# Justin900429/autonomous_driving_with_diffusion_model

Hardware: AMD Instinct MI355X
Metric: denoising-steps/sec (higher is better)
Workload: dtype f32

## Files before the change

### autonomous_driving_with_diffusion_model_amd/_lib.py

```python
from __future__ import annotations

import ctypes as C
import os
from typing import Optional, Sequence

import torch

_HERE = os.path.dirname(os.path.abspath(__file__))
LIB_PATH = os.environ.get("ADX_LIB") or os.path.join(_HERE, "libadx.so")

c_f32p = C.POINTER(C.c_float)
i32, i64, f32, vp = C.c_int32, C.c_int64, C.c_float, C.c_void_p


class TConvDesc(C.Structure):
    _fields_ = [("kind", i32), ("taps", i32), ("stride", i32), ("pad", i32), ("c0", i32), ("c1", i32),
                ("cout", i32), ("lin", i32), ("lout", i32), ("groups", i32), ("eps", f32), ("w_layout", i32),
                ("w_flip", i32), ("exact", i32), ("lin_valid", i32), ("lout_valid", i32)]


class TConvIO(C.Structure):
    _fields_ = [("x0", vp), ("x0_sb", i64), ("x0_sc", i64), ("x0_sl", i64),
                ("x1", vp), ("x1_sb", i64), ("x1_sc", i64), ("x1_sl", i64),
                ("packed_w", vp), ("bias", vp), ("gamma", vp), ("beta", vp),
# ... 204 lines not shown
    "adx_control_reset": (i32, [vp, i32, i32, i32, vp, vp]),
    "adx_traj_metrics": (i32, [C.POINTER(MetricsCfg), vp, vp, vp, vp, vp, vp, vp, vp, vp, vp, vp]),
    "adx_metrics_state_bytes": (C.c_size_t, []),
    "adx_metrics_reset": (i32, [vp, vp]),
    "adx_metrics_accumulate": (i32, [vp, vp, vp, vp, vp, vp, vp, i32, i32, vp]),
    "adx_noise_normal": (i32, [vp, i32, i64, vp, i64, vp]),
    "adx_noise_words": (i32, [vp, i32, i64, vp, i64, vp]),
    "adx_noise_advance": (i32, [vp, vp]),
    "adx_warm_init": (i32, [vp, i32, vp, vp, i32, i32, i32, i32, f32, f32, vp, i64, i32, vp]),
    "adx_add_noise": (i32, [vp, vp, vp, vp, vp, i32, vp, i32, i32, i32, i32, vp]),
}

_LAZY_SIGS = {
    "adx_resnet_plan_grids": (i32, [vp, i32, i32, i32, i32, i32, i32, C.POINTER(i32), C.POINTER(i32), i32]),
    "adx_conv2d_hs3x3q_walk": (i32, [i32, i32, i32, C.POINTER(i32), C.POINTER(i32)]),
    "adx_conv2d_pack_ds": (i32, [i32, i32, vp, vp, vp]),
    "adx_conv2d_block_s2_cells": (i32, [i32, i32, vp, vp, vp, vp, vp, vp, vp, vp, vp, i32, i32, i32, i32, vp]),
    "adx_ddim_step_pin": (i32, [C.POINTER(StepCoef), vp, vp, vp, vp, i32, i64, C.POINTER(PinDesc), vp, vp, i32, i32, i32, vp]),
    "adx_ddpm_step_pin": (i32, [C.POINTER(StepCoef), vp, vp, vp, vp, i32, i64, C.POINTER(PinDesc), vp, vp, i32, i32, i32, vp]),
    "adx_dpm_step_pin": (i32, [C.POINTER(DpmCoef), vp, vp, vp, vp, i32, i64, C.POINTER(PinDesc), vp, vp, i32, i32, i32, vp]),
    "adx_pin_apply": (i32, [vp, C.POINTER(PinDesc), vp, i64, i32, i32, i32, vp]),
    "adx_cost_field_from_occupancy": (i32, [vp, vp, i32, i32, i32, f32, f32, f32, i32, i32, vp]),
    "adx_capsules_from_boxes": (i32, [vp, vp, i32, i32, f32, vp]),
    "adx_stop_short": (i32, [vp, C.POINTER(GuideDesc), C.POINTER(FieldDesc), C.POINTER(RouteDesc), C.POINTER(CapsuleDesc), vp, i32, vp, vp,
                             vp, vp, vp, i32, i32, i32, vp]),
    "adx_traj_modes": (i32, [C.POINTER(ModesCfg), vp, vp, vp, vp, vp, vp, vp, vp]),
    "adx_commit_state_bytes": (C.c_size_t, [i32, i32]),
    "adx_commit_reset": (i32, [vp, i32, i32, vp, vp]),
    "adx_traj_commit": (i32, [C.POINTER(CommitCfg), vp, vp, vp, vp, vp, vp, vp, vp, vp, vp, vp, vp, vp]),
}
# ... 116 lines not shown
```

### autonomous_driving_with_diffusion_model_amd/csrc/adx_common.h

```cpp
#pragma once
#include <atomic>
#include <mutex>
#include <hip/hip_runtime.h>
#include <stdint.h>
#include <stdio.h>
#include <string.h>

#include "../../include/adx.h"
#include "plan.h"

namespace adx {

void set_error(const char* fmt, ...);

#define ADX_CHECK_HIP(expr)                                                              \
  do {                                                                                   \
    hipError_t _e = (expr);                                                              \
    if (_e != hipSuccess) {                                                              \
      adx::set_error("%s failed: %s (%s:%d)", #expr, hipGetErrorString(_e), __FILE__, __LINE__); \
      return ADX_ERR_HIP;                                                                \
    }                                                                                    \
  } while (0)

#define ADX_REQUIRE(cond, ...)                                                           \
// ... 15 lines not shown

struct DebugSwitches {
  bool conv_exact = false;
  bool wgrad_exact = false;
  bool tconv_exact = false;
  bool unet_chain = true;
  unsigned chain_mask = ~0u;
  bool unet_pipe = true;
  bool conv_vrow = true;
  bool conv_cells = true;
  int train_cells = 5;
  int hs_mode = -1;
  bool wgrad_deterministic = false;
  bool hs_dma = true;
  bool hs_s2q = true;
  bool hs_persist = true;
  int hs_reserve_cus = -1;
  int hs_grid_cap = 0;
  int resnet_streams = 2;
  int resnet_split_from = -1;
  bool check_range = false;
};
const DebugSwitches& debug_switches();

struct DeviceOnce {
  std::atomic<uint64_t>& done;
  uint64_t bit = 0;
  bool owner = false;
  static std::mutex& mu() { static std::mutex m; return m; }
  explicit DeviceOnce(std::atomic<uint64_t>& d) : done(d) {
// ... 54 lines not shown
```

### autonomous_driving_with_diffusion_model_amd/csrc/api.cpp

```cpp
#include <stdarg.h>
#include <stdlib.h>

#include "sched.h"
#include "tconv.h"

namespace adx {

static thread_local char g_err[512] = "";

void set_error(const char* fmt, ...) {
  va_list ap;
  va_start(ap, fmt);
  vsnprintf(g_err, sizeof(g_err), fmt, ap);
  va_end(ap);
}

static thread_local PlanSink* t_plan_sink = nullptr;
PlanSink* plan_sink() { return t_plan_sink; }
void plan_set_sink(PlanSink* s) { t_plan_sink = s; }

int plan_emit(PlanSink* s, const PlanLaunch& l) {
  ADX_REQUIRE(s->n < s->cap, "plan export: more than %d launches", s->cap);
  s->rec[s->n++] = l;
  return ADX_OK;
// ... 11 lines not shown
const DebugSwitches& debug_switches() {
  static const DebugSwitches sw = [] {
    DebugSwitches d;
    auto is = [](const char* name, char v) { const char* e = getenv(name); return e != nullptr && e[0] == v && e[1] == '\0'; };
    d.conv_exact = is("ADX_CONV_EXACT", '1');
    d.wgrad_exact = is("ADX_WGRAD_EXACT", '1');
    d.tconv_exact = is("ADX_TCONV_EXACT", '1');
    d.unet_chain = !is("ADX_UNET_CHAIN", '0');
    d.unet_pipe = !is("ADX_UNET_PIPE", '0');
    d.conv_cells = !is("ADX_CONV_CELLS", '0');
    d.conv_vrow = !is("ADX_CONV_VROW", '0');
    d.train_cells = is("ADX_TRAIN_CELLS", '0') ? 0 : (is("ADX_TRAIN_CELLS", '1') ? 1 : (is("ADX_TRAIN_CELLS", '2') ? 2 : (is("ADX_TRAIN_CELLS", '3') ? 3 : (is("ADX_TRAIN_CELLS", '4') ? 4 : 5))));
    d.check_range = is("ADX_CHECK_RANGE", '1');
    d.hs_dma = !is("ADX_HS_DMA", '0');
    d.hs_persist = !is("ADX_HS_PERSIST", '0');
    d.hs_s2q = !is("ADX_HS_S2Q", '0');
    d.wgrad_deterministic = is("ADX_WGRAD_DETERMINISTIC", '1');
    if (const char* e = getenv("ADX_CHAIN_MASK")) d.chain_mask = (unsigned)strtoul(e, nullptr, 0);
    if (const char* e = getenv("ADX_HS_MODE")) d.hs_mode = atoi(e);
    if (const char* e = getenv("ADX_HS_RESERVE_CUS")) d.hs_reserve_cus = atoi(e) < 0 ? 0 : (atoi(e) & ~7);
    if (const char* e = getenv("ADX_HS_GRID_CAP")) d.hs_grid_cap = atoi(e) < 8 ? 0 : (atoi(e) & ~7);
    if (const char* e = getenv("ADX_RESNET_SPLIT_FROM")) d.resnet_split_from = atoi(e) < 0 ? -1 : atoi(e);
    if (const char* e = getenv("ADX_RESNET_STREAMS")) d.resnet_streams = atoi(e) < 1 ? 1 : (atoi(e) > 4 ? 4 : atoi(e));
    return d;
  }();
  return sw;
}

int embed_forward(const adx_embed_weights* w, int dim, const int64_t* t, int t_rows, const float* cond,
                  const float* feat, int feat_rows, int rows, float* time_embed, float* mish_cond, hipStream_t s);
// ... 360 lines not shown
```

### autonomous_driving_with_diffusion_model_amd/csrc/conv2d.hip

```cpp
#include <stdlib.h>

#include <vector>

#include "adx_common.h"
#include "conv2d_internal.h"

namespace adx {

constexpr int kCoutT = 64;
constexpr size_t kMaxLds = 96 * 1024;

template <int STRIDE, int K, int ROWS, int CCH = 16>
__global__ void __launch_bounds__(256) conv2d_kernel(const Conv2dArgs a) {
  constexpr int TH = 4 * ROWS;
  constexpr int CC = (K == 7) ? 4 : CCH;
  constexpr int PH = (TH - 1) * STRIDE + K;
  constexpr int PW = (kTileW - 1) * STRIDE + K;
  constexpr int PLANE = PH * PW;
  constexpr int NP = CC * PLANE;
  constexpr int PITEMS = (NP + 255) / 256;
  constexpr int NTAPS = K * K;
  constexpr int NW4 = NTAPS * CC * (kCoutT / 4);
  constexpr int WITEMS = (NW4 + 255) / 256;
  extern __shared__ __attribute__((aligned(16))) float smem[];
// ... 897 lines not shown
  const int Q = grid / 8;
  int n = 0;
  for (int b = 0; b < grid; ++b) {
    const HsQWalk wk = hs3x3q_walk(b & 7, b >> 3, units);
    counts[b] = 0;
    for (int u = wk.first; u < wk.end; u += Q, ++counts[b], ++n) {
      ADX_REQUIRE(n < units, "adx_conv2d_hs3x3q_walk: internal error (more visits than units)");
      const HsQUnit un = hs3x3q_unit(u, cout_tiles);
      visits[2 * n] = un.sp;
      visits[2 * n + 1] = un.ct;
    }
  }
  return ADX_OK;
}

static int resnet_forward_impl(adx_resnet* r, const void* packed, void* workspace, const float* img,
                               const uint8_t* frames_u8, const float* mean, const float* stdv, int32_t batch, int32_t h,
                               int32_t w, float* feature, adx_stream stream);

int adx_resnet_forward(adx_resnet* r, const void* packed, void* workspace, const float* img, int32_t batch, int32_t h,
                       int32_t w, float* feature, adx_stream stream) {
  ADX_REQUIRE(img != nullptr, "adx_resnet_forward: null image");
  return resnet_forward_impl(r, packed, workspace, img, nullptr, nullptr, nullptr, batch, h, w, feature, stream);
}

int adx_resnet_forward_u8(adx_resnet* r, const void* packed, void* workspace, const uint8_t* frames_hwc, const float* mean,
                          const float* stdv, int32_t batch, int32_t h, int32_t w, float* feature, adx_stream stream) {
  ADX_REQUIRE(frames_hwc && mean && stdv, "adx_resnet_forward_u8: null frames / mean / std");
  return resnet_forward_impl(r, packed, workspace, nullptr, frames_hwc, mean, stdv, batch, h, w, feature, stream);
}
// ... 158 lines not shown
```

### autonomous_driving_with_diffusion_model_amd/csrc/conv2d_hs.hip

```cpp
#include <type_traits>
#include <stdlib.h>

#include "adx_common.h"
#include "conv2d_internal.h"
#include "conv2d_hs_common.h"

namespace adx {

template <bool AFFINE = true>
__device__ __forceinline__ void cells_store32(float (&v)[16], const float* sc, const float* sh, int cl0, const float (*res8)[8],
                                              bool relu, __amdgpu_buffer_rsrc_t yrsrc, uint32_t vcell, uint32_t so, uint32_t cplane,
                                              float& amax) {
  float lm = 0.f;
#pragma unroll
  for (int i = 0; i < 2; ++i)
#pragma unroll
    for (int j = 0; j < 4; ++j) {
      const auto sw = __builtin_amdgcn_permlane32_swap(f2u(v[8 * i + j]), f2u(v[8 * i + 4 + j]), false, false);
      v[8 * i + j] = u2f(sw[0]);
      v[8 * i + 4 + j] = u2f(sw[1]);
    }
#pragma unroll
  for (int i = 0; i < 2; ++i) {
    float o[8];
// ... 343 lines not shown
  if (threadIdx.x == 0 && blockIdx.x < 16384) g_hs_trace[blockIdx.x * 8 + slot] = __builtin_readcyclecounter();
}
__device__ __forceinline__ void hs_trace_id() {
  if (threadIdx.x == 0 && blockIdx.x < 16384) {
    unsigned hw, xcc;
    asm volatile("s_getreg_b32 %0, hwreg(HW_REG_HW_ID)" : "=s"(hw));
    asm volatile("s_getreg_b32 %0, hwreg(HW_REG_XCC_ID)" : "=s"(xcc));
    g_hs_trace[blockIdx.x * 8 + 7] = ((unsigned long long)xcc << 32) | hw;
  }
}
#define HS_TRACE(slot) hs_trace(slot)
#else
#define HS_TRACE(slot)
#endif

template <int MODE, int STATS = 0, bool XCELLS = false, bool YCELLS = false, bool VR = false>
__global__ void __launch_bounds__(MODE == 0 ? 256 : 512, 2) conv2d_hs3x3_kernel(const Conv2dArgs a) {
  constexpr bool VROW = YCELLS || VR;
  constexpr int NT = MODE == 0 ? 256 : 512;
  constexpr int TH = MODE == 1 ? 16 : 8;
  constexpr int CT = MODE == 2 ? 2 : 1;
  constexpr int K = 3, PH = TH + 2, PW = 34, PLANE = PH * PW, NITEM = 2 * PLANE;
  constexpr int PIT = (NITEM + NT - 1) / NT;
  constexpr int NW = 9 * 256, WST = 3 * 256 * CT;
  constexpr int WIT = (WST + NT - 1) / NT;
  static_assert(PIT <= K, "a patch slice travels with each stage of a chunk");
  extern __shared__ __attribute__((aligned(16))) unsigned char smem_raw[];
  u32x4* patch = reinterpret_cast<u32x4*>(smem_raw);
  u32x4* wl = patch + 2 * 4 * PLANE;
  float* ss = reinterpret_cast<float*>(wl + 2 * WST);
  u32x4* dummy = reinterpret_cast<u32x4*>(ss + 2 * 64 * CT + 8);
  float* bsl = reinterpret_cast<float*>(dummy + 3);
  const int tid = threadIdx.x, lane = tid & 63;
  const int wave = __builtin_amdgcn_readfirstlane(tid >> 6);
  const int rowpair = MODE == 2 ? (wave & 3) : wave, slab = MODE == 2 ? (wave >> 2) : 0;
#ifdef ADX_HS_TRACE
  hs_trace_id();
#endif
  HS_TRACE(0);
// ... 1 lines not shown
  {
    const int per = gridDim.x >> 3;
    if (bid < per * 8) bid = (bid & 7) * per + (bid >> 3);
  }
  int kpart = 0;
  if (a.ksplit > 1) { kpart = bid % a.ksplit; bid /= a.ksplit; }
  const int ct = bid % a.cout_tiles; bid /= a.cout_tiles;
  const int tx = bid % a.tiles_x; bid /= a.tiles_x;
  const int ty = bid % a.tiles_y; bid /= a.tiles_y;
  const int n = VROW ? 0 : bid;
  const int oy0 = ty * TH, ox0 = tx * kTileW;
  const int iy0 = oy0 - a.pad, ix0 = ox0 - a.pad;
  const int cout0 = (ct * CT + slab) * kHsCout;
  const int l31 = lane & 31, khalf = lane >> 5;
  const int vx0 = tx * kTileW;
  const int vl = vx0 + l31;
  auto vdiv = [&](int v) { return (int)(((float)v + 0.5f) * a.inv_vw); };
  const int nl = VROW ? vdiv(vl) : 0, xl = VROW ? vl - nl * a.vw : 0;
  const bool lane_valid = !VROW || (nl < a.N && xl < a.W);
  const size_t hw = (size_t)a.H * a.W;
  const int nchunks_all = a.cin_pad / kHsCC;
  const int nchunks = a.ksplit > 1 ? a.cper : nchunks_all;
  const int chunk0 = kpart * nchunks;
  const float* xin = a.x + ((size_t)n * a.Cin + (size_t)chunk0 * kHsCC) * hw;
  const int nstages = nchunks * K;
  const u32x4* wsrc = reinterpret_cast<const u32x4*>(a.w) + ((size_t)ct * CT * nchunks_all + chunk0) * NW;
  constexpr uint32_t kOutside = 0xC0000000u;
  const __amdgpu_buffer_rsrc_t xrsrc = __builtin_amdgcn_make_buffer_rsrc(
      const_cast<float*>(xin), 0,
      (int)(uint32_t)((VROW ? (size_t)a.N * a.Cin : (size_t)(a.Cin - chunk0 * kHsCC)) * hw * sizeof(float)), 0x00020000);
  const uint32_t plane_bytes = (uint32_t)(hw * sizeof(float));
// ... 67 lines not shown
      xs_inv = __builtin_bit_cast(float, (uint32_t)(127 - sh) << 23);
    }
  }

  f32x16 accm[2][2], accl[2][2];
#pragma unroll
  for (int r = 0; r < 2; ++r)
#pragma unroll
    for (int m = 0; m < 2; ++m)
#pragma unroll
      for (int i = 0; i < 16; ++i) { accm[r][m][i] = 0.f; accl[r][m][i] = 0.f; }

  u32x4 wv[2][WIT];
  float pv[2][8];
  auto load_w = [&](int stage, int set) {
    const u32x4* ws = wsrc + (size_t)stage * 768;
#pragma unroll
    for (int k = 0; k < WIT; ++k) wv[set][k] = ws[wsrc_off[k]];
  };
  auto store_w = [&](int set, int buf) {
#pragma unroll
    for (int k = 0; k < WIT; ++k) {
      u32x4* d = (WST % NT == 0 || wdst[k] >= 0) ? wl + buf * WST + wdst[k] : dummy + 2;
      *d = wv[set][k];
    }
  };
  auto load_p = [&](int chunk, int k, int set) {
    const uint32_t cbase = (uint32_t)chunk * kHsCC * plane_bytes;
    if (XCELLS) {
      const u32x4 h4 = __builtin_amdgcn_raw_buffer_load_b128(xrsrc, goff[k], cbase, 0);
// ... 13 lines not shown
    u32x4 hi, lo;
    if (XCELLS) {
#pragma unroll
      for (int j = 0; j < 4; ++j) {
        hi[j] = __builtin_bit_cast(uint32_t, pv[set][j]);
        lo[j] = __builtin_bit_cast(uint32_t, pv[set][4 + j]);
      }
    } else {
      split8(pv[set], xs, hi, lo);
    }
    u32x4* pd = patch + buf * 4 * PLANE + pcell[k];
    u32x4* d0 = pcell[k] >= 0 ? pd : dummy;
    u32x4* d1 = pcell[k] >= 0 ? pd + PLANE : dummy + 1;
    *d0 = hi;
    *d1 = lo;
  };

  const int pb_lane = khalf * 2 * PLANE + (rowpair * 2) * PW + l31;
  const int wa_lane = slab * 768 + khalf * 64 + l31;

  load_w(0, 0);
  store_w(0, 0);
#pragma unroll
  for (int k = 0; k < PIT; ++k) { load_p(0, k, 0); store_p(0, k, 0); }
  load_w(1, 1);
  if (tid < 2 * 64 * CT) ss[tid] = ssv;
  if (STATS == 2 && tid < 4 * 64 * CT) bsl[tid] = bsv;
  load_p(1, 0, 1);
  HS_TRACE(1);
  __syncthreads();
  HS_TRACE(2);

  for (int cp = 0; cp < nchunks; cp += 2) {
#pragma unroll
    for (int i = 0; i < 6; ++i) {
      const int s = 3 * cp + i;
      const int kh = i % 3, cpar = (i / 3) & 1;
      const u32x4* pb0 = patch + cpar * 4 * PLANE + pb_lane;
      const u32x4* wa0 = wl + (i & 1) * WST + wa_lane;
      load_w(s + 2 < nstages ? s + 2 : nstages - 1, i & 1);
      if ((i + 1) % 3 < PIT) load_p(s + 4 < nstages ? (s + 4) / 3 : nchunks - 1, (i + 1) % 3, i & 1);
      __builtin_amdgcn_sched_barrier(0);
#pragma unroll
      for (int kw = 0; kw < K; ++kw) {
        f16x8 A[2][2], B[2][2];
#pragma unroll
        for (int pl = 0; pl < 2; ++pl) {
// ... 8 lines not shown
          for (int m = 0; m < 2; ++m) {
            accm[r][m] = hs_mfma(A[0][m], B[0][r], accm[r][m]);
            accl[r][m] = hs_mfma(A[0][m], B[1][r], accl[r][m]);
            accl[r][m] = hs_mfma(A[1][m], B[0][r], accl[r][m]);
          }
        if (kw == 0) {
          store_w((i + 1) & 1, (i + 1) & 1);
          if (i % 3 < PIT) store_p((i + 1) & 1, i % 3, ((i + 3) / 3) & 1);
        }
      }
      __syncthreads();
    }
  }

  HS_TRACE(3);
  const int ox = VROW ? xl : ox0 + l31;
  const uint32_t plane_ob = (uint32_t)(a.OH * a.OW) * (uint32_t)sizeof(float);
  const size_t img = (size_t)n * a.Cout * a.OH * a.OW;
  const int img_bytes = (int)(uint32_t)((VROW ? (uint32_t)a.N : 1u) * (uint32_t)a.Cout * plane_ob);
  const uint32_t img_off = VROW ? (uint32_t)nl * (uint32_t)a.Cout * plane_ob : 0u;
  float* const ybase = a.ksplit > 1 ? a.part + (size_t)kpart * a.part_stride : a.y;
  const __amdgpu_buffer_rsrc_t yrsrc = __builtin_amdgcn_make_buffer_rsrc(ybase + img, 0, img_bytes, 0x00020000);
  const __amdgpu_buffer_rsrc_t rrsrc = __builtin_amdgcn_make_buffer_rsrc(
      const_cast<float*>(a.res != nullptr ? a.res + img : a.y), 0, a.res != nullptr ? img_bytes : 0, 0x00020000);
  const float* sst = ss + slab * 64;
  const uint32_t cbase_o = (uint32_t)cout0 * plane_ob;
  const uint32_t cplane = (uint32_t)(a.OH * a.OW) * 16u;
  const uint32_t cell0 = (uint32_t)(cout0 >> 3) * 2u * cplane;
  bool inside[2];
  uint32_t pix[2];
#pragma unroll
  for (int rr = 0; rr < 2; ++rr) {
    const int oy = oy0 + rowpair * 2 + rr;
    inside[rr] = lane_valid && oy < a.OH && ox < a.OW;
    pix[rr] = (uint32_t)(oy * a.OW + ox);
  }
  auto half4 = [](uint32_t h0, uint32_t h1, uint32_t l0, uint32_t l1, float* out) {
    const float inv = 1.f / kLoScale;
    asm("v_fma_mix_f32 %0, %1, %2, %3 op_sel:[0,0,0] op_sel_hi:[1,0,1]" : "=v"(out[0]) : "v"(l0), "s"(inv), "v"(h0));
    asm("v_fma_mix_f32 %0, %1, %2, %3 op_sel:[1,0,1] op_sel_hi:[1,0,1]" : "=v"(out[1]) : "v"(l0), "s"(inv), "v"(h0));
    asm("v_fma_mix_f32 %0, %1, %2, %3 op_sel:[0,0,0] op_sel_hi:[1,0,1]" : "=v"(out[2]) : "v"(l1), "s"(inv), "v"(h1));
    asm("v_fma_mix_f32 %0, %1, %2, %3 op_sel:[1,0,1] op_sel_hi:[1,0,1]" : "=v"(out[3]) : "v"(l1), "s"(inv), "v"(h1));
  };
  float amax = 0.f;
  if constexpr (YCELLS) {
    const uint32_t khoff = (uint32_t)khalf * 2u * cplane;
    uint32_t vcell[2], vres[2];
#pragma unroll
    for (int rr = 0; rr < 2; ++rr) {
      vcell[rr] = inside[rr] ? img_off + pix[rr] * 16u + khoff : kOutside;
      vres[rr] = !inside[rr] ? kOutside : a.res_cells ? vcell[rr] : img_off + pix[rr] * 4u + (uint32_t)(8 * khalf) * plane_ob;
    }
    uint32_t rraw[2][2][2][8];
#pragma unroll
    for (int rr = 0; rr < 2; ++rr)
#pragma unroll
      for (int half = 0; half < 2; ++half)
#pragma unroll
// ... 867 lines not shown
  }
  const float sc = scale != nullptr ? scale[c] : 1.f, sh = shift != nullptr ? shift[c] : 0.f;
  v = v * sc + sh;
  if (res != nullptr) v += reinterpret_cast<const f32x4*>(res)[i];
  if (relu) {
#pragma unroll
    for (int k = 0; k < 4; ++k) v[k] = __builtin_fmaxf(v[k], 0.f);
  }
  reinterpret_cast<f32x4*>(y)[i] = v;
  float amax = 0.f;
#pragma unroll
  for (int k = 0; k < 4; ++k) amax = fp16_amax(amax, v[k]);
  range_flag(status, out_of_fp16(amax));
}

static constexpr size_t hs3x3_lds(int mode, int stats) {
  const int th = mode == 1 ? 16 : 8, ct = mode == 2 ? 2 : 1;
  return (size_t)2 * 64 * (th + 2) * 34 + (size_t)2 * 3 * 256 * ct * 16 + (2 * 64 * ct + 8) * sizeof(float) + 48 +
         (stats == 2 ? 4 * 64 * ct * sizeof(float) : 0);
}
static_assert(hs3x3_lds(0, 2) <= 80 * 1024 && hs3x3_lds(1, 2) <= 160 * 1024 && hs3x3_lds(2, 2) <= 160 * 1024, "LDS budget");

Hs3x3Plan conv2d_hs3x3_plan(const ConvSpec& L, const Hs3x3Query& q, const DebugSwitches& sw) {
  Hs3x3Plan p;
  p.admitted = q.fmt == 0;
  if (!hs_eligible(L, sw) || !(L.k == 3 && L.stride == 1 && L.pad == 1) || (L.cin_pad / kHsCC) % 2 != 0) return p;
  const int N = q.N, OH = q.H, OW = q.W, nchunks = L.cin_pad / kHsCC;
  int mode = L.cin < 256 ? 0 : (OH > 8 ? 1 : (L.cout % 128 == 0 ? 2 : 0));
  const long grid0 = (long)N * ceil_div(OH, 8) * ceil_div(OW, kTileW) * (L.cout / kHsCout);
  if (grid0 <= 256) mode = 0;
  if (sw.hs_mode >= 0 && !(sw.hs_mode == 2 && L.cout % 128 != 0)) mode = sw.hs_mode == 1 || sw.hs_mode == 2 ? sw.hs_mode : 0;
  const int th = mode == 1 ? 16 : 8, ct = mode == 2 ? 2 : 1;
  const bool xc = (q.fmt & kFmtXCells) != 0, yc = (q.fmt & kFmtYCells) != 0, rc = (q.fmt & kFmtResCells) != 0 && q.has_res;
  const bool xscaled = q.x_scale == kXScalePre;
  const bool in_ok = (size_t)N * L.cin * q.H * q.W * sizeof(float) < 0xC0000000u;
  const bool bytes_ok = in_ok && (size_t)N * L.cout * OH * OW * sizeof(float) < 0xC0000000u;
// ... 26 lines not shown
  if (!stats && split_shape && q.split_floats > 0 && q.x_scale == kXScaleNone && (OH * OW) % 4 == 0 && q.y_aligned && (!q.has_res || q.res_aligned)) {
    const size_t out_floats = (size_t)N * L.cout * OH * OW;
    int S = 16;
    while (S > 1 && (nchunks % S != 0 || (nchunks / S) % 2 != 0 || p.grid * S > 256 || out_floats * S > q.split_floats)) S >>= 1;
    if (S > 1) { p.ksplit = S; p.cper = nchunks / S; p.grid *= S; }
  }
  const bool cells_out = !stats && p.ksplit == 1 && (xc || yc || rc) && !(xc && xscaled && !yc && !rc);
  if (stats ? q_train || q_dgrad : cells_out && q_plain) {
    p.family = kHs3x3q; p.dma = sw.hs_dma; p.threads = kQNT;
    p.lds = p.dma ? kQLdsD : kQLds;
    p.vw = vw; p.tiles_x = vtiles_x; p.tiles_y = ceil_div(OH, kQTH); p.cout_tiles = L.cout / 128;
    p.q_slots = hs3x3q_slots(p.cout_tiles * p.tiles_x * p.tiles_y, q.cus, sw.hs_dma && sw.hs_persist);
    p.grid = (size_t)8 * p.q_slots;
    return p;
  }
  p.lds = hs3x3_lds(mode, p.stats);
  if (p.ksplit > 1) return p;
  p.xcells = xc; p.ycells = cells_out;
  p.vr = !cells_out && (!(xc || yc || rc) || ((stats || xscaled) && !yc && !rc)) && vrow_ok;
  if (p.ycells || p.vr) {
    p.vw = vw; p.tiles_x = vtiles_x;
    p.grid = (size_t)p.cout_tiles * p.tiles_x * p.tiles_y;
  }
  return p;
}

typedef void (*HsKernel)(const Conv2dArgs);

template <int MODE>
static const HsKernel* hs3x3_kernels() {
#define HS_K(S, X, Y, V) &conv2d_hs3x3_kernel<MODE, S, X, Y, V>
  static const HsKernel table[3 * 8] = {
      HS_K(0, false, false, false), HS_K(0, false, false, true), HS_K(0, false, true, false), nullptr,
      HS_K(0, true, false, false),  HS_K(0, true, false, true),  HS_K(0, true, true, false),  nullptr,
      HS_K(1, false, false, false), HS_K(1, false, false, true), nullptr, nullptr,
      HS_K(1, true, false, false),  HS_K(1, true, false, true),  nullptr, nullptr,
      HS_K(2, false, false, false), HS_K(2, false, false, true), nullptr, nullptr,
      HS_K(2, true, false, false),  HS_K(2, true, false, true),  nullptr, nullptr};
#undef HS_K
  return table;
}

static int hs3x3_launch(const Hs3x3Plan& p, Conv2dArgs a, hipStream_t s) {
  const HsKernel* const table = p.mode == 1 ? hs3x3_kernels<1>() : (p.mode == 2 ? hs3x3_kernels<2>() : hs3x3_kernels<0>());
  static std::atomic<uint64_t> attr[3];
  if (DeviceOnce once{attr[p.mode]}; once) {
    for (int v = 0; v < 3 * 8; ++v)
      if (table[v] != nullptr)
        ADX_CHECK_HIP(hipFuncSetAttribute(reinterpret_cast<const void*>(table[v]), hipFuncAttributeMaxDynamicSharedMemorySize,
                                          (int)hs3x3_lds(p.mode, v / 8)));
    once.commit();
  }
  ADX_REQUIRE(p.grid < (1u << 31), "conv2d_hs: grid too large");
  ADX_REQUIRE((size_t)a.Cout * a.OH * a.OW * sizeof(float) < 0x7FFFFFFFu, "conv2d_hs: one image of the output exceeds the 32-bit byte offsets");
  if (p.ycells) {
    ADX_REQUIRE(a.y_cells && a.x_amax == nullptr, "conv2d_hs: cell-layout operands come with a cell-layout output (and no dynamic range)");
    ADX_REQUIRE((long)a.N * p.vw < (1L << 21), "conv2d_hs: batch x width exceeds the virtual-row arithmetic");
    ADX_REQUIRE((size_t)a.N * a.Cout * a.OH * a.OW * sizeof(float) < 0xC0000000u && (size_t)a.N * a.Cin * a.H * a.W * sizeof(float) < 0xC0000000u,
                "conv2d_hs: a cell-layout tensor exceeds the 32-bit byte offsets");
  } else if (p.xcells) {
    ADX_REQUIRE(p.stats == 0 || ((a.x_amax == nullptr || a.x_amax_n < 0) && (a.bs_raw == nullptr) == (a.x_amax == nullptr) && !a.y_cells && !a.res_cells),
                "conv2d_hs: a cell-layout input with statistics belongs to a training-forward launch or to a data gradient with its scale");
    ADX_REQUIRE((size_t)a.N * a.Cin * a.H * a.W * sizeof(float) < 0xC0000000u, "conv2d_hs: a cell-layout tensor exceeds the 32-bit byte offsets");
  }
  a.tiles_x = p.tiles_x; a.tiles_y = p.tiles_y; a.cout_tiles = p.cout_tiles;
  a.vw = p.vw; a.inv_vw = 1.f / (float)p.vw;
  a.ksplit = p.ksplit; a.cper = p.cper;
// ... 95 lines not shown
```

### autonomous_driving_with_diffusion_model_amd/csrc/conv2d_internal.h

```cpp
#pragma once
#include <algorithm>
#include <vector>

#include "adx_common.h"

namespace adx {

constexpr int kTileH = 4;
constexpr int kTileW = 32;

struct ConvSpec {
  int cin, cout, k, stride, pad;
  int t_w, t_g, t_b, t_m, t_v;
  size_t o_w, o_scale, o_shift;
  int cin_pad, cc;
  int fuse_with;
  int dgrad;
};

struct Conv2dArgs {
  const float* x;
  const float* w;
  const float* scale;
  const float* shift;
// ... 74 lines not shown
};
struct Hs3x3Plan {
  bool admitted = false;
  int family = kHsNone;
  int mode = 0;
  int stats = 0;
  bool xcells = false, ycells = false, vr = false;
  bool dma = false;
  int ksplit = 1, cper = 0;
  int tiles_x = 0, tiles_y = 0, cout_tiles = 0, vw = 0, q_slots = 0;
  size_t grid = 0;
  int threads = 0;
  size_t lds = 0;
  int stats_tiles = 0;
  size_t stats_need = 0;
};
Hs3x3Plan conv2d_hs3x3_plan(const ConvSpec& L, const Hs3x3Query& q, const DebugSwitches& sw = debug_switches());
struct HsQWalk { int first, end; };
__host__ __device__ inline HsQWalk hs3x3q_walk(int xcd, int slot, int units) {
  return HsQWalk{(int)(((long)xcd * units) >> 3) + slot, (int)(((long)(xcd + 1) * units) >> 3)};
}
struct HsQUnit { int sp, ct; };
__host__ __device__ inline HsQUnit hs3x3q_unit(int u, int cout_tiles) {
  const int sp = u / cout_tiles;
  return HsQUnit{sp, u - sp * cout_tiles};
}
inline int hs3x3q_slots(int units, int cus, bool persistent) {
  const int longest = (units + 7) / 8;
  return persistent ? std::min(longest, std::max(1, cus / 8)) : longest;
}
inline bool conv2d_hs3x3_plain(const ConvSpec& L, int N, int H, int W) {
// ... 130 lines not shown
```

### include/adx.h

```cpp
#ifndef ADX_H
#define ADX_H

#include <stddef.h>
#include <stdint.h>

#ifdef __cplusplus
extern "C" {
#endif

#define ADX_OK 0
#define ADX_ERR_INVALID (-1)
#define ADX_ERR_HIP (-2)
#define ADX_ERR_STATE (-3)
#define ADX_ERR_RANGE (-4)

typedef void* adx_stream;

int adx_version(void);
const char* adx_source_hash(void);
const char* adx_last_error(void);


typedef struct adx_tconv_desc {
  int32_t kind, taps, stride, pad;
// ... 132 lines not shown
int adx_resnet_forward(adx_resnet* r, const void* packed, void* workspace, const float* img ,
                       int32_t batch, int32_t h, int32_t w, float* feature , adx_stream s);
int adx_resnet_forward_u8(adx_resnet* r, const void* packed, void* workspace, const uint8_t* frames_hwc,
                          const float* mean , const float* stdv , int32_t batch, int32_t h, int32_t w,
                          float* feature , adx_stream s);
#define ADX_RESNET_PLAN_INTS 24
#define ADX_RESNET_PLAN_CAPTURING 1
enum { ADX_RESNET_PLAN_STEM_POOL = 0, ADX_RESNET_PLAN_STEM = 1, ADX_RESNET_PLAN_MAXPOOL = 2, ADX_RESNET_PLAN_CONV = 3,
       ADX_RESNET_PLAN_ENTRY = 4, ADX_RESNET_PLAN_AVGPOOL_FC = 5 };
int adx_resnet_plan_describe(const adx_resnet* r, int32_t batch, int32_t h, int32_t w, int32_t flags, int32_t* n_records, int32_t* ints,
                             int32_t max_records);
#define ADX_RESNET_GRID_INTS 6
int adx_resnet_plan_grids(const adx_resnet* r, int32_t batch, int32_t h, int32_t w, int32_t flags, int32_t cus, int32_t reserve,
                          int32_t* n_records, int32_t* ints, int32_t max_records);
int adx_conv2d_hs3x3q_walk(int32_t units, int32_t cout_tiles, int32_t grid, int32_t* counts, int32_t* visits);
int32_t adx_resnet_status_words(const adx_resnet* r);
int adx_resnet_set_status(adx_resnet* r, uint32_t* words );
const char* adx_resnet_status_name(const adx_resnet* r, int32_t group);

typedef struct adx_conv2d_desc { int32_t cin, cout, k, stride, pad; } adx_conv2d_desc;
size_t adx_conv2d_packed_bytes(const adx_conv2d_desc* d);
int adx_conv2d_pack(const adx_conv2d_desc* d, const float* w , float* packed, adx_stream s);
int adx_conv2d_forward(const adx_conv2d_desc* d, const float* x, const float* packed_w, const float* scale,
                       const float* shift, const float* res, float* y, int32_t n, int32_t h, int32_t w,
                       int32_t relu, adx_stream s);
int adx_conv2d_cells_supported(const adx_conv2d_desc* d, int32_t n, int32_t h, int32_t w);
int adx_conv2d_forward_cells(const adx_conv2d_desc* d, const void* x, const float* packed_w, const float* scale,
                             const float* shift, const void* res, void* y, int32_t n, int32_t h, int32_t w, int32_t relu,
                             int32_t fmt, adx_stream s);
int adx_conv2d_pack_ds(int32_t cin, int32_t cout, const float* w, float* packed, adx_stream s);
int adx_conv2d_block_s2_cells(int32_t cin, int32_t cout, const void* x, const float* packed_w1, const float* scale1,
                              const float* shift1, void* y1, const float* packed_wd, const float* scaled, const float* shiftd,
                              void* yd, int32_t n, int32_t h, int32_t w, int32_t flags, adx_stream s);
int adx_conv2d_stem_pool(const void* x, int32_t x_u8, const float* packed_w, const float* scale, const float* shift,
                         const float* mean, const float* stdv, void* y, int32_t n, int32_t h, int32_t w, int32_t y_cells,
                         adx_stream s);
size_t adx_conv2d_wgrad_scratch_bytes(void);
int adx_conv2d_wgrad(const adx_conv2d_desc* d, const float* x, const float* dy, float* dw, int32_t n, int32_t h,
                     int32_t w, void* scratch, adx_stream s);
int adx_conv2d_wgrad_ex(const adx_conv2d_desc* d, const float* x, const float* dy, float* dw, int32_t n, int32_t h,
                        int32_t w, void* scratch, int32_t estimate_range, adx_stream s);
// ... 366 lines not shown
```

Before: 173.8.

## Add paired-chunk 16x16 MFMA form of the hs3x3 conv main loop

```diff
diff --git a/autonomous_driving_with_diffusion_model_amd/_lib.py b/autonomous_driving_with_diffusion_model_amd/_lib.py
--- a/autonomous_driving_with_diffusion_model_amd/_lib.py
+++ b/autonomous_driving_with_diffusion_model_amd/_lib.py
@@ -242,6 +242,8 @@
 _LAZY_SIGS = {
     "adx_resnet_plan_grids": (i32, [vp, i32, i32, i32, i32, i32, i32, C.POINTER(i32), C.POINTER(i32), i32]),
     "adx_conv2d_hs3x3q_walk": (i32, [i32, i32, i32, C.POINTER(i32), C.POINTER(i32)]),
+    "adx_conv2d_hs3x3_pair_walk": (i32, [i32, C.POINTER(i32), C.POINTER(i32), i32]),
+    "adx_conv2d_hs3x3_plan_query": (i32, [C.POINTER(Conv2dDesc), i32, i32, i32, i32, i32, C.POINTER(i32)]),
     "adx_conv2d_pack_ds": (i32, [i32, i32, vp, vp, vp]),
     "adx_conv2d_block_s2_cells": (i32, [i32, i32, vp, vp, vp, vp, vp, vp, vp, vp, vp, i32, i32, i32, i32, vp]),
     "adx_ddim_step_pin": (i32, [C.POINTER(StepCoef), vp, vp, vp, vp, i32, i64, C.POINTER(PinDesc), vp, vp, i32, i32, i32, vp]),
diff --git a/autonomous_driving_with_diffusion_model_amd/csrc/adx_common.h b/autonomous_driving_with_diffusion_model_amd/csrc/adx_common.h
--- a/autonomous_driving_with_diffusion_model_amd/csrc/adx_common.h
+++ b/autonomous_driving_with_diffusion_model_amd/csrc/adx_common.h
@@ -53,6 +53,7 @@
   bool wgrad_deterministic = false;
   bool hs_dma = true;
   bool hs_s2q = true;
+  bool hs_pair = true;
   bool hs_persist = true;
   int hs_reserve_cus = -1;
   int hs_grid_cap = 0;
diff --git a/autonomous_driving_with_diffusion_model_amd/csrc/api.cpp b/autonomous_driving_with_diffusion_model_amd/csrc/api.cpp
--- a/autonomous_driving_with_diffusion_model_amd/csrc/api.cpp
+++ b/autonomous_driving_with_diffusion_model_amd/csrc/api.cpp
@@ -49,6 +49,7 @@
     d.check_range = is("ADX_CHECK_RANGE", '1');
     d.hs_dma = !is("ADX_HS_DMA", '0');
     d.hs_persist = !is("ADX_HS_PERSIST", '0');
+    d.hs_pair = !is("ADX_HS_PAIR", '0');
     d.hs_s2q = !is("ADX_HS_S2Q", '0');
     d.wgrad_deterministic = is("ADX_WGRAD_DETERMINISTIC", '1');
     if (const char* e = getenv("ADX_CHAIN_MASK")) d.chain_mask = (unsigned)strtoul(e, nullptr, 0);
diff --git a/autonomous_driving_with_diffusion_model_amd/csrc/conv2d.hip b/autonomous_driving_with_diffusion_model_amd/csrc/conv2d.hip
--- a/autonomous_driving_with_diffusion_model_amd/csrc/conv2d.hip
+++ b/autonomous_driving_with_diffusion_model_amd/csrc/conv2d.hip
@@ -935,6 +935,57 @@
   return ADX_OK;
 }
 
+int adx_conv2d_hs3x3_pair_walk(int32_t nchunks, int32_t* n_events, int32_t* events, int32_t max_events) {
+  ADX_REQUIRE(n_events && events && nchunks >= 2 && nchunks % 2 == 0 && max_events >= 1, "adx_conv2d_hs3x3_pair_walk: %d chunks, room for %d events",
+              nchunks, max_events);
+  const int npairs = nchunks / 2, nstages = 9 * npairs;
+  int n = 0;
+  auto put = [&](int stage, int kind, int chunk, int tr, int cb, int rs, int idle) {
+    if (n < max_events) {
+      const int32_t e[ADX_PAIR_EVENT_INTS] = {stage, kind, chunk, tr, cb, rs, idle};
+      memcpy(events + (size_t)n * ADX_PAIR_EVENT_INTS, e, sizeof(e));
+    }
+    ++n;
+  };
+  put(-1, ADX_PAIR_FETCH_W, -1, -1, -1, 0, 0);
+  put(-1, ADX_PAIR_WRITE_W, -1, -1, 0, 0, 0);
+  for (int k = 0; k < 3; ++k) { put(-1, ADX_PAIR_FETCH_P, 0, k, -1, -1, 0); put(-1, ADX_PAIR_WRITE_P, 0, k, 0, -1, 0); }
+  put(-1, ADX_PAIR_FETCH_W, -1, -1, -1, 1, 0);
+  put(-1, ADX_PAIR_FETCH_P, 1, 0, -1, -1, 0);
+  for (int pair = 0; pair < npairs; ++pair)
+    for (int i = 0; i < 9; ++i) {
+      const int s = 9 * pair + i;
+      const HsPairStage st = hs_pair_stage(i), nx = hs_pair_stage((i + 1) % 9);
+      put(s, ADX_PAIR_FETCH_W, -1, -1, -1, s + 2 < nstages ? s + 2 : nstages - 1, s + 2 >= nstages);
+      if (nx.pround >= 0) {
+        const int c = 2 * pair + 1 + (i == 8 ? 2 : nx.pnext);
+        put(s, ADX_PAIR_FETCH_P, c < nchunks ? c : nchunks - 1, nx.pround, -1, -1, c >= nchunks);
+      }
+      for (int t = 0; t < 2; ++t)
+        put(s, ADX_PAIR_READ, 2 * pair + st.tap[t].odd, st.tap[t].kh * 3 + i % 3, st.tap[t].odd, hs_pair_run(pair, i, t) / 256, s & 1);
+      put(s, ADX_PAIR_WRITE_W, -1, -1, (s + 1) & 1, s + 1 < nstages ? s + 1 : nstages - 1, s + 1 >= nstages);
+      if (st.pround >= 0) {
+        const int c = 2 * pair + 1 + st.pnext;
+        put(s, ADX_PAIR_WRITE_P, c < nchunks ? c : nchunks - 1, st.pround, st.pnext ? 0 : 1, -1, c >= nchunks);
+      }
+    }
+  *n_events = n;
+  ADX_REQUIRE(n <= max_events, "adx_conv2d_hs3x3_pair_walk: %d events, room for %d", n, max_events);
+  return ADX_OK;
+}
+
+int adx_conv2d_hs3x3_plan_query(const adx_conv2d_desc* d, int32_t n, int32_t h, int32_t w, int32_t fmt, int32_t has_res, int32_t* out) {
+  ConvSpec L;
+  const int rc = spec_from_desc(d, &L);
+  if (rc != ADX_OK) return rc;
+  ADX_REQUIRE(out && n >= 1 && h >= 1 && w >= 1 && fmt >= 0 && fmt <= 7, "adx_conv2d_hs3x3_plan_query: n %d, %d x %d, fmt %d", n, h, w, fmt);
+  Hs3x3Query q;
+  q.N = n; q.H = h; q.W = w; q.fmt = fmt; q.affine = true; q.relu = true; q.has_res = has_res != 0; q.cus = 256;
+  const Hs3x3Plan p = L.k == 3 && L.stride == 1 ? conv2d_hs3x3_plan(L, q) : Hs3x3Plan{};
+  out[0] = p.family; out[1] = p.mode; out[2] = p.ksplit; out[3] = p.pair ? 1 : 0; out[4] = p.admitted ? 1 : 0;
+  return ADX_OK;
+}
+
 static int resnet_forward_impl(adx_resnet* r, const void* packed, void* workspace, const float* img,
                                const uint8_t* frames_u8, const float* mean, const float* stdv, int32_t batch, int32_t h,
                                int32_t w, float* feature, adx_stream stream);
diff --git a/autonomous_driving_with_diffusion_model_amd/csrc/conv2d_hs.hip b/autonomous_driving_with_diffusion_model_amd/csrc/conv2d_hs.hip
--- a/autonomous_driving_with_diffusion_model_amd/csrc/conv2d_hs.hip
+++ b/autonomous_driving_with_diffusion_model_amd/csrc/conv2d_hs.hip
@@ -381,15 +381,16 @@
 #define HS_TRACE(slot)
 #endif
 
-template <int MODE, int STATS = 0, bool XCELLS = false, bool YCELLS = false, bool VR = false>
+template <int MODE, int STATS = 0, bool XCELLS = false, bool YCELLS = false, bool VR = false, bool PAIR = false>
 __global__ void __launch_bounds__(MODE == 0 ? 256 : 512, 2) conv2d_hs3x3_kernel(const Conv2dArgs a) {
+  static_assert(!PAIR || (MODE == 0 && STATS == 0), "the PAIR form is the plain 4-wave tile");
   constexpr bool VROW = YCELLS || VR;
   constexpr int NT = MODE == 0 ? 256 : 512;
   constexpr int TH = MODE == 1 ? 16 : 8;
   constexpr int CT = MODE == 2 ? 2 : 1;
   constexpr int K = 3, PH = TH + 2, PW = 34, PLANE = PH * PW, NITEM = 2 * PLANE;
   constexpr int PIT = (NITEM + NT - 1) / NT;
-  constexpr int NW = 9 * 256, WST = 3 * 256 * CT;
+  constexpr int NW = 9 * 256, WST = PAIR ? 2 * 256 : 3 * 256 * CT;
   constexpr int WIT = (WST + NT - 1) / NT;
   static_assert(PIT <= K, "a patch slice travels with each stage of a chunk");
   extern __shared__ __attribute__((aligned(16))) unsigned char smem_raw[];
@@ -421,7 +422,8 @@
   const int cout0 = (ct * CT + slab) * kHsCout;
   const int l31 = lane & 31, khalf = lane >> 5;
   const int vx0 = tx * kTileW;
-  const int vl = vx0 + l31;
+  const int ecol = PAIR ? 16 * ((lane >> 4) & 1) + (lane & 15) : l31;
+  const int vl = vx0 + ecol;
   auto vdiv = [&](int v) { return (int)(((float)v + 0.5f) * a.inv_vw); };
   const int nl = VROW ? vdiv(vl) : 0, xl = VROW ? vl - nl * a.vw : 0;
   const bool lane_valid = !VROW || (nl < a.N && xl < a.W);
@@ -519,6 +521,11 @@
   u32x4 wv[2][WIT];
   float pv[2][8];
   auto load_w = [&](int stage, int set) {
+    if constexpr (PAIR) {
+#pragma unroll
+      for (int k = 0; k < 2; ++k) wv[set][k] = wsrc[hs_pair_run(0, stage, k) + tid];
+      return;
+    }
     const u32x4* ws = wsrc + (size_t)stage * 768;
 #pragma unroll
     for (int k = 0; k < WIT; ++k) wv[set][k] = ws[wsrc_off[k]];
@@ -562,6 +569,14 @@
     u32x4* d1 = pcell[k] >= 0 ? pd + PLANE : dummy + 1;
     *d0 = hi;
     *d1 = lo;
+  };
+
+  auto half4 = [](uint32_t h0, uint32_t h1, uint32_t l0, uint32_t l1, float* out) {
+    const float inv = 1.f / kLoScale;
+    asm("v_fma_mix_f32 %0, %1, %2, %3 op_sel:[0,0,0] op_sel_hi:[1,0,1]" : "=v"(out[0]) : "v"(l0), "s"(inv), "v"(h0));
+    asm("v_fma_mix_f32 %0, %1, %2, %3 op_sel:[1,0,1] op_sel_hi:[1,0,1]" : "=v"(out[1]) : "v"(l0), "s"(inv), "v"(h0));
+    asm("v_fma_mix_f32 %0, %1, %2, %3 op_sel:[0,0,0] op_sel_hi:[1,0,1]" : "=v"(out[2]) : "v"(l1), "s"(inv), "v"(h1));
+    asm("v_fma_mix_f32 %0, %1, %2, %3 op_sel:[1,0,1] op_sel_hi:[1,0,1]" : "=v"(out[3]) : "v"(l1), "s"(inv), "v"(h1));
   };
 
   const int pb_lane = khalf * 2 * PLANE + (rowpair * 2) * PW + l31;
@@ -579,6 +594,170 @@
   __syncthreads();
   HS_TRACE(2);
 
+  if constexpr (PAIR) {
+    const int j = lane & 15, kq = lane >> 4, ts = kq >> 1, kh2 = kq & 1;
+    const int npairs = nchunks >> 1;
+    f32x4 am[4][4], al[4][4];
+#pragma unroll
+    for (int cb = 0; cb < 4; ++cb)
+#pragma unroll
+      for (int pb = 0; pb < 4; ++pb)
+#pragma unroll
+        for (int i = 0; i < 4; ++i) { am[cb][pb][i] = 0.f; al[cb][pb][i] = 0.f; }
+    const u32x4* pb_g[3];
+#pragma unroll
+    for (int g = 0; g < 3; ++g) {
+      const HsPairTap t0 = hs_pair_stage(3 * g).tap[0], t1 = hs_pair_stage(3 * g).tap[1];
+      pb_g[g] = patch + kh2 * 2 * PLANE + (rowpair * 2) * PW + j + (ts ? t1.odd * 4 * PLANE + t1.kh * PW : t0.odd * 4 * PLANE + t0.kh * PW);
+    }
+    const int wa_pair = ts * 256 + kh2 * 64 + j;
+    auto load_runs = [&](int o0, int o1, int set) {
+      wv[set][0] = wsrc[o0 + tid];
+      wv[set][1] = wsrc[o1 + tid];
+    };
+    auto pair_stages = [&](const int par, const int pair) __attribute__((always_inline)) {
+      const bool more = pair + 1 < npairs;
+#pragma unroll
+      for (int i = 0; i < 9; ++i) {
+        const int gp = (i + par) & 1;
+        const HsPairStage st = hs_pair_stage(i), nx = hs_pair_stage((i + 1) % 9);
+        if (i + 2 < 9) load_runs(hs_pair_run(pair, i + 2, 0), hs_pair_run(pair, i + 2, 1), gp);
+        else load_runs(more ? hs_pair_run(pair + 1, i + 2 - 9, 0) : hs_pair_run(pair, 8, 0), more ? hs_pair_run(pair + 1, i + 2 - 9, 1) : hs_pair_run(pair, 8, 1), gp);
+        if (nx.pround >= 0) {
+          const int c = 2 * pair + 1 + (i == 8 ? 2 : nx.pnext);
+          load_p(c < nchunks ? c : nchunks - 1, nx.pround, gp);
+        }
+        __builtin_amdgcn_sched_barrier(0);
+        const u32x4* pb0 = pb_g[i / 3] + i % 3;
+        const u32x4* wa0 = wl + gp * WST + wa_pair;
+        f16x8 A[2][4], B[2][4];
+#pragma unroll
+        for (int pl = 0; pl < 2; ++pl) {
+#pragma unroll
+          for (int cb = 0; cb < 4; ++cb) A[pl][cb] = __builtin_bit_cast(f16x8, wa0[pl * 128 + cb * 16]);
+#pragma unroll
+          for (int pb = 0; pb < (XCELLS ? 4 : 2); ++pb) B[pl][pb] = __builtin_bit_cast(f16x8, pb0[pl * PLANE + (pb >> 1) * PW + (pb & 1) * 16]);
+        }
+#pragma unroll
+        for (int pb = 0; pb < 4; ++pb) {
+          if (!XCELLS && pb == 1) {
+            __builtin_amdgcn_sched_barrier(0);
+#pragma unroll
+            for (int pl = 0; pl < 2; ++pl)
+#pragma unroll
+              for (int q = 2; q < 4; ++q) B[pl][q] = __builtin_bit_cast(f16x8, pb0[pl * PLANE + (q >> 1) * PW + (q & 1) * 16]);
+          }
+#pragma unroll
+          for (int cb = 0; cb < 4; ++cb) {
+            am[cb][pb] = __builtin_amdgcn_mfma_f32_16x16x32_f16(A[0][cb], B[0][pb], am[cb][pb], 0, 0, 0);
+            al[cb][pb] = __builtin_amdgcn_mfma_f32_16x16x32_f16(A[0][cb], B[1][pb], al[cb][pb], 0, 0, 0);
+          }
+#pragma unroll
+          for (int cb = 0; cb < 4; ++cb) al[cb][pb] = __builtin_amdgcn_mfma_f32_16x16x32_f16(A[1][cb], B[0][pb], al[cb][pb], 0, 0, 0);
+          if (pb == (XCELLS ? 0 : 1)) {
+            store_w(gp ^ 1, gp ^ 1);
+            if (st.pround >= 0) store_p(gp ^ 1, st.pround, st.pnext ? 0 : 1);
+          }
+        }
+        __syncthreads();
+      }
+    };
+    int pair = 0;
+    for (; pair + 1 < npairs; pair += 2) {
+      pair_stages(0, pair);
+      pair_stages(1, pair + 1);
+    }
+    if (pair < npairs) pair_stages(0, pair);
+
+    const int ox = VROW ? xl : ox0 + ecol;
+    const uint32_t plane_ob = (uint32_t)(a.OH * a.OW) * (uint32_t)sizeof(float);
+    const uint32_t cplane = (uint32_t)(a.OH * a.OW) * 16u;
+    const size_t img = (size_t)n * a.Cout * a.OH * a.OW;
+    const int img_bytes = (int)(uint32_t)((VROW ? (uint32_t)a.N : 1u) * (uint32_t)a.Cout * plane_ob);
+    const uint32_t img_off = VROW ? (uint32_t)nl * (uint32_t)a.Cout * plane_ob : 0u;
+    const __amdgpu_buffer_rsrc_t yrsrc = __builtin_amdgcn_make_buffer_rsrc(a.y + img, 0, img_bytes, 0x00020000);
+    const __amdgpu_buffer_rsrc_t rrsrc = __builtin_amdgcn_make_buffer_rsrc(
+        const_cast<float*>(a.res != nullptr ? a.res + img : a.y), 0, a.res != nullptr ? img_bytes : 0, 0x00020000);
+    const uint32_t cbase_o = (uint32_t)cout0 * plane_ob;
+    const uint32_t cell0 = (uint32_t)(cout0 >> 3) * 2u * cplane;
+    const bool rcells = YCELLS && a.res_cells;
+    bool inside[2];
+    uint32_t vout[2], vres[2];
+#pragma unroll
+    for (int rr = 0; rr < 2; ++rr) {
+      const int oy = oy0 + rowpair * 2 + rr;
+      inside[rr] = lane_valid && oy < a.OH && ox < a.OW;
+      const uint32_t pix = (uint32_t)(oy * a.OW + ox);
+      const uint32_t vc = img_off + pix * 16u + (uint32_t)ts * 2u * cplane, vf = img_off + pix * 4u + (uint32_t)(8 * ts) * plane_ob;
+      vout[rr] = !inside[rr] ? kOutside : (YCELLS ? vc : vf);
+      vres[rr] = !inside[rr] ? kOutside : (rcells ? vc : vf);
+    }
+    uint32_t rraw[4][2][8];
+#pragma unroll
+    for (int cb = 0; cb < 4; ++cb)
+#pragma unroll
+      for (int rr = 0; rr < 2; ++rr) {
+        if (rcells) {
+          const uint32_t so = cell0 + (uint32_t)(2 * cb) * 2u * cplane;
+          const u32x4 h4 = __builtin_amdgcn_raw_buffer_load_b128(rrsrc, vres[rr], so, 0);
+          const u32x4 l4 = __builtin_amdgcn_raw_buffer_load_b128(rrsrc, vres[rr], so + cplane, 0);
+#pragma unroll
+          for (int c = 0; c < 4; ++c) { rraw[cb][rr][c] = h4[c]; rraw[cb][rr][4 + c] = l4[c]; }
+        } else {
+#pragma unroll
+          for (int c = 0; c < 8; ++c)
+            rraw[cb][rr][c] = __builtin_amdgcn_raw_buffer_load_b32(rrsrc, vres[rr], cbase_o + (uint32_t)(16 * cb + c) * plane_ob, 0);
+        }
+      }
+    float amax = 0.f;
+#pragma unroll
+    for (int cb = 0; cb < 4; ++cb)
+#pragma unroll
+      for (int rr = 0; rr < 2; ++rr) {
+        float o[8], r8[8];
+#pragma unroll
+        for (int i = 0; i < 4; ++i) {
+          const int cl = 16 * cb + 4 * kq + i;
+          float x = (am[cb][2 * rr][i] + al[cb][2 * rr][i] * (1.f / kLoScale)) * xs_inv;
+          float y = (am[cb][2 * rr + 1][i] + al[cb][2 * rr + 1][i] * (1.f / kLoScale)) * xs_inv;
+          x = x * ss[cl] + ss[64 + cl];
+          y = y * ss[cl] + ss[64 + cl];
+          const auto sw = __builtin_amdgcn_permlane16_swap(f2u(x), f2u(y), false, false);
+          o[i] = u2f(sw[0]);
+          o[4 + i] = u2f(sw[1]);
+        }
+        if (rcells) {
+          half4(rraw[cb][rr][0], rraw[cb][rr][1], rraw[cb][rr][4], rraw[cb][rr][5], r8);
+          half4(rraw[cb][rr][2], rraw[cb][rr][3], rraw[cb][rr][6], rraw[cb][rr][7], r8 + 4);
+        } else {
+#pragma unroll
+          for (int c = 0; c < 8; ++c) r8[c] = u2f(rraw[cb][rr][c]);
+        }
+        float lm = 0.f;
+#pragma unroll
+        for (int c = 0; c < 8; ++c) {
+          const float t = o[c] + r8[c];
+          o[c] = a.relu ? __builtin_fmaxf(t, 0.f) : t;
+          lm = fp16_amax(lm, o[c]);
+        }
+        amax = fp16_amax(amax, inside[rr] ? lm : 0.f);
+        if constexpr (YCELLS) {
+          u32x4 hi, lo;
+          split8(o, 1.f, hi, lo);
+          const uint32_t so = cell0 + (uint32_t)(2 * cb) * 2u * cplane;
+          __builtin_amdgcn_raw_buffer_store_b128(hi, yrsrc, vout[rr], so, 0);
+          __builtin_amdgcn_raw_buffer_store_b128(lo, yrsrc, vout[rr], so + cplane, 0);
+          asm volatile("s_nop 0" ::"v"(hi), "v"(lo));
+        } else {
+#pragma unroll
+          for (int c = 0; c < 8; ++c)
+            __builtin_amdgcn_raw_buffer_store_b32(f2u(o[c]), yrsrc, vout[rr], cbase_o + (uint32_t)(16 * cb + c) * plane_ob, 0);
+        }
+      }
+    range_flag(a.status, out_of_fp16(amax));
+    return;
+  }
+
   for (int cp = 0; cp < nchunks; cp += 2) {
 #pragma unroll
     for (int i = 0; i < 6; ++i) {
@@ -617,7 +796,7 @@
   }
 
   HS_TRACE(3);
-  const int ox = VROW ? xl : ox0 + l31;
+  const int ox = VROW ? xl : ox0 + ecol;
   const uint32_t plane_ob = (uint32_t)(a.OH * a.OW) * (uint32_t)sizeof(float);
   const size_t img = (size_t)n * a.Cout * a.OH * a.OW;
   const int img_bytes = (int)(uint32_t)((VROW ? (uint32_t)a.N : 1u) * (uint32_t)a.Cout * plane_ob);
@@ -638,13 +817,6 @@
     inside[rr] = lane_valid && oy < a.OH && ox < a.OW;
     pix[rr] = (uint32_t)(oy * a.OW + ox);
   }
-  auto half4 = [](uint32_t h0, uint32_t h1, uint32_t l0, uint32_t l1, float* out) {
-    const float inv = 1.f / kLoScale;
-    asm("v_fma_mix_f32 %0, %1, %2, %3 op_sel:[0,0,0] op_sel_hi:[1,0,1]" : "=v"(out[0]) : "v"(l0), "s"(inv), "v"(h0));
-    asm("v_fma_mix_f32 %0, %1, %2, %3 op_sel:[1,0,1] op_sel_hi:[1,0,1]" : "=v"(out[1]) : "v"(l0), "s"(inv), "v"(h0));
-    asm("v_fma_mix_f32 %0, %1, %2, %3 op_sel:[0,0,0] op_sel_hi:[1,0,1]" : "=v"(out[2]) : "v"(l1), "s"(inv), "v"(h1));
-    asm("v_fma_mix_f32 %0, %1, %2, %3 op_sel:[1,0,1] op_sel_hi:[1,0,1]" : "=v"(out[3]) : "v"(l1), "s"(inv), "v"(h1));
-  };
   float amax = 0.f;
   if constexpr (YCELLS) {
     const uint32_t khoff = (uint32_t)khalf * 2u * cplane;
@@ -1542,12 +1714,13 @@
   range_flag(status, out_of_fp16(amax));
 }
 
-static constexpr size_t hs3x3_lds(int mode, int stats) {
+static constexpr size_t hs3x3_lds(int mode, int stats, bool pair = false) {
   const int th = mode == 1 ? 16 : 8, ct = mode == 2 ? 2 : 1;
-  return (size_t)2 * 64 * (th + 2) * 34 + (size_t)2 * 3 * 256 * ct * 16 + (2 * 64 * ct + 8) * sizeof(float) + 48 +
+  return (size_t)2 * 64 * (th + 2) * 34 + (size_t)2 * (pair ? 2 : 3 * ct) * 256 * 16 + (2 * 64 * ct + 8) * sizeof(float) + 48 +
          (stats == 2 ? 4 * 64 * ct * sizeof(float) : 0);
 }
 static_assert(hs3x3_lds(0, 2) <= 80 * 1024 && hs3x3_lds(1, 2) <= 160 * 1024 && hs3x3_lds(2, 2) <= 160 * 1024, "LDS budget");
+static_assert(hs3x3_lds(0, 0, true) <= 80 * 1024, "LDS budget: two workgroups of the PAIR form per CU");
 
 Hs3x3Plan conv2d_hs3x3_plan(const ConvSpec& L, const Hs3x3Query& q, const DebugSwitches& sw) {
   Hs3x3Plan p;
@@ -1604,7 +1777,8 @@
     p.grid = (size_t)8 * p.q_slots;
     return p;
   }
-  p.lds = hs3x3_lds(mode, p.stats);
+  p.pair = sw.hs_pair && sw.hs_mode < 0 && mode == 0 && p.ksplit == 1 && !stats;
+  p.lds = hs3x3_lds(mode, p.stats, p.pair);
   if (p.ksplit > 1) return p;
   p.xcells = xc; p.ycells = cells_out;
   p.vr = !cells_out && (!(xc || yc || rc) || ((stats || xscaled) && !yc && !rc)) && vrow_ok;
@@ -1631,16 +1805,25 @@
   return table;
 }
 
+static const HsKernel* hs3x3_pair_kernels() {
+#define HS_K(X, Y, V) &conv2d_hs3x3_kernel<0, 0, X, Y, V, true>
+  static const HsKernel table[8] = {HS_K(false, false, false), HS_K(false, false, true), HS_K(false, true, false), nullptr,
+                                    HS_K(true, false, false),  HS_K(true, false, true),  HS_K(true, true, false),  nullptr};
+#undef HS_K
+  return table;
+}
+
 static int hs3x3_launch(const Hs3x3Plan& p, Conv2dArgs a, hipStream_t s) {
-  const HsKernel* const table = p.mode == 1 ? hs3x3_kernels<1>() : (p.mode == 2 ? hs3x3_kernels<2>() : hs3x3_kernels<0>());
-  static std::atomic<uint64_t> attr[3];
-  if (DeviceOnce once{attr[p.mode]}; once) {
-    for (int v = 0; v < 3 * 8; ++v)
+  const HsKernel* const table = p.pair ? hs3x3_pair_kernels() : (p.mode == 1 ? hs3x3_kernels<1>() : (p.mode == 2 ? hs3x3_kernels<2>() : hs3x3_kernels<0>()));
+  static std::atomic<uint64_t> attr[4];
+  if (DeviceOnce once{attr[p.pair ? 3 : p.mode]}; once) {
+    for (int v = 0; v < (p.pair ? 8 : 3 * 8); ++v)
       if (table[v] != nullptr)
         ADX_CHECK_HIP(hipFuncSetAttribute(reinterpret_cast<const void*>(table[v]), hipFuncAttributeMaxDynamicSharedMemorySize,
-                                          (int)hs3x3_lds(p.mode, v / 8)));
+                                          (int)hs3x3_lds(p.mode, v / 8, p.pair)));
     once.commit();
   }
+  ADX_REQUIRE(!p.pair || (p.mode == 0 && p.stats == 0 && p.ksplit == 1), "conv2d_hs: the PAIR form is the plain 4-wave tile (internal error)");
   ADX_REQUIRE(p.grid < (1u << 31), "conv2d_hs: grid too large");
   ADX_REQUIRE((size_t)a.Cout * a.OH * a.OW * sizeof(float) < 0x7FFFFFFFu, "conv2d_hs: one image of the output exceeds the 32-bit byte offsets");
   if (p.ycells) {
diff --git a/autonomous_driving_with_diffusion_model_amd/csrc/conv2d_internal.h b/autonomous_driving_with_diffusion_model_amd/csrc/conv2d_internal.h
--- a/autonomous_driving_with_diffusion_model_amd/csrc/conv2d_internal.h
+++ b/autonomous_driving_with_diffusion_model_amd/csrc/conv2d_internal.h
@@ -112,7 +112,20 @@
   size_t lds = 0;
   int stats_tiles = 0;
   size_t stats_need = 0;
-};
+  bool pair = false;
+};
+struct HsPairTap { int odd, kh; };
+struct HsPairStage {
+  HsPairTap tap[2];
+  int pround;
+  int pnext;
+};
+__host__ __device__ constexpr HsPairStage hs_pair_stage(int i) {
+  return i < 3 ? HsPairStage{{{0, 0}, {0, 1}}, i, 0} : (i < 6 ? HsPairStage{{{0, 2}, {1, 0}}, -1, 0} : HsPairStage{{{1, 1}, {1, 2}}, i - 6, 1});
+}
+__host__ __device__ constexpr int hs_pair_run(int pair, int i, int t) {
+  return ((2 * pair + hs_pair_stage(i).tap[t].odd) * 9 + hs_pair_stage(i).tap[t].kh * 3 + i % 3) * 256;
+}
 Hs3x3Plan conv2d_hs3x3_plan(const ConvSpec& L, const Hs3x3Query& q, const DebugSwitches& sw = debug_switches());
 struct HsQWalk { int first, end; };
 __host__ __device__ inline HsQWalk hs3x3q_walk(int xcd, int slot, int units) {
diff --git a/include/adx.h b/include/adx.h
--- a/include/adx.h
+++ b/include/adx.h
@@ -170,6 +170,9 @@
 int adx_resnet_plan_grids(const adx_resnet* r, int32_t batch, int32_t h, int32_t w, int32_t flags, int32_t cus, int32_t reserve,
                           int32_t* n_records, int32_t* ints, int32_t max_records);
 int adx_conv2d_hs3x3q_walk(int32_t units, int32_t cout_tiles, int32_t grid, int32_t* counts, int32_t* visits);
+#define ADX_PAIR_EVENT_INTS 7
+enum { ADX_PAIR_READ = 0, ADX_PAIR_FETCH_P = 1, ADX_PAIR_WRITE_P = 2, ADX_PAIR_FETCH_W = 3, ADX_PAIR_WRITE_W = 4 };
+int adx_conv2d_hs3x3_pair_walk(int32_t nchunks, int32_t* n_events, int32_t* events, int32_t max_events);
 int32_t adx_resnet_status_words(const adx_resnet* r);
 int adx_resnet_set_status(adx_resnet* r, uint32_t* words );
 const char* adx_resnet_status_name(const adx_resnet* r, int32_t group);
@@ -181,6 +184,7 @@
                        const float* shift, const float* res, float* y, int32_t n, int32_t h, int32_t w,
                        int32_t relu, adx_stream s);
 int adx_conv2d_cells_supported(const adx_conv2d_desc* d, int32_t n, int32_t h, int32_t w);
+int adx_conv2d_hs3x3_plan_query(const adx_conv2d_desc* d, int32_t n, int32_t h, int32_t w, int32_t fmt, int32_t has_res, int32_t* out);
 int adx_conv2d_forward_cells(const adx_conv2d_desc* d, const void* x, const float* packed_w, const float* scale,
                              const float* shift, const void* res, void* y, int32_t n, int32_t h, int32_t w, int32_t relu,
                              int32_t fmt, adx_stream s);
```

New measurement: 176.1, median of 6. 1.01x the previous value.
